# PeterFWS/Structure-PLP-SLAM

Hardware: NVIDIA H100
Metric: frames_per_sec_extract_match_poseopt (higher is better)
Workload: dtype u8/f64

## Files before the change

### structure-plp-slam_b200/csrc/local_map.cu

```cuda
#include "common.cuh"
#include "local_map_kernels.cuh"
#include "match_kernels.cuh"
#include "pose_kernels.cuh"
#include "tracker.h"

namespace plp {

namespace {

using lm::LocalDev;
using lm::local_finish_kernel;
using lm::local_gather_kernel;
using lm::local_observe_kernel;
using lm::local_prep_kernel;

}

}

using namespace plp;

extern "C" {

plp_status plp_tracker_reserve_local_map(plp_tracker *t, float log_scale_factor, int max_local_points) {
// ... 71 lines not shown
    D.rb = t->standing(kStageRobust);
    if (from_update) {
        D.kf.local_idx = D.rb.local_idx = t->upd_local_idx;
        D.kf.local_idx_offsets = D.rb.local_idx_offsets = t->upd_local_idx_offsets;
    }
    D.pos_w = local->pos_w;
    D.normal = local->obs_mean_normal;
    D.min_d = local->min_valid_dist;
    D.max_d = local->max_valid_dist;
    D.max_raw = local->max_valid_dist_raw;
    D.lm_desc = local->desc;
    D.valid = local->valid;
    D.offsets = local->offsets;
    D.margin = margin;
    D.matched = d_matched_out;
    D.local = d_local_out;
    D.observable = d_observable_out;
    D.pose = d_pose_out;
    D.num_tracked = d_num_tracked_out;
    D.n_inliers = d_n_inliers_out;
    D.lm_iters = d_lm_iters_out;
    D.status = d_status_out;

    PLP_LAUNCH(ctx, local_prep_kernel, batch, lm::kThreads, 0, D);
    PLP_CHECK_LAUNCH();
    const dim3 ogrid(div_up(t->max_local, lm::kObserveThreads), batch);
    PLP_LAUNCH(ctx, local_observe_kernel, ogrid, lm::kObserveThreads, 0, D);
    PLP_CHECK_LAUNCH();
    PLP_TRY(launch_point_match(ctx, D.mjobs, batch, t->cap > kMatchMaxPoints ? kMatchMaxPoints : t->cap, t->grid, 1,
                               lm::kLoweRatio, 0));
    PLP_LAUNCH(ctx, local_gather_kernel, batch, lm::kThreads, 0, D);
    PLP_CHECK_LAUNCH();
    plp_pose_opt_cfg cfg{4, 10};
    PLP_TRY(launch_pose_opt(ctx, D.posejobs, batch, t->cam, cfg));
    PLP_LAUNCH(ctx, local_finish_kernel, batch, lm::kThreads, 0, D);
    PLP_CHECK_LAUNCH();
    return PLP_OK;
}

plp_status plp_tracker_match_counts(const plp_tracker *t, const uint32_t **d_motion, const uint32_t **d_local) {
    PLP_REQUIRE(t && d_motion && d_local, "null pointer");
    *d_motion = t->dev.num_matches;
    *d_local = t->local ? t->local->num_matches : nullptr;
    return PLP_OK;
}

}
```

### structure-plp-slam_b200/csrc/match.cu

```cuda
#include "match_common.cuh"
#include "match_kernels.cuh"
#include "point_match_kernels.cuh"
#include "detmath.h"

namespace plp {

namespace {

constexpr int kThreads = 512;
__global__ void hamming_matrix_kernel(const uint8_t *__restrict__ a, int na, const uint8_t *__restrict__ b,
                                      int nb, uint16_t *__restrict__ out) {
    __shared__ uint4 sb[32][2];
    const int j0 = blockIdx.x * 32, i0 = blockIdx.y * 32;
    const int tx = threadIdx.x, ty = threadIdx.y;
    if (ty < 2 && j0 + tx < nb) sb[tx][ty] = __ldg(reinterpret_cast<const uint4 *>(b + 32 * (size_t)(j0 + tx)) + ty);
    __syncthreads();
    for (int r = ty; r < 32; r += 8) {
        const int i = i0 + r;
        if (i >= na) break;
        uint4 a0, a1;
        load_desc(a + 32 * (size_t)i, a0, a1);
        if (j0 + tx < nb) out[(size_t)i * nb + j0 + tx] = (uint16_t)hamming256(a0, a1, sb[tx][0], sb[tx][1]);
    }
}
// ... 407 lines not shown
            if (lane >= off) incl += nb;
        }
        int run = incl - local, med = 0x7fffffff;
#pragma unroll
        for (int q = 0; q < 9; ++q) {
            if (med == 0x7fffffff && run <= rank && rank < run + cnt[q]) med = lane * 9 + q;
            run += cnt[q];
        }
        for (int off = 16; off >= 1; off >>= 1) med = min(med, __shfl_xor_sync(0xffffffffu, med, off));
        if ((unsigned)med < best_median) {
            best_median = (unsigned)med;
            best_idx = i;
        }
        __syncwarp();
    }
    if (lane == 0) best_out[lm] = best_idx;
}

}

plp_status launch_point_match(plp_ctx *ctx, const PointMatchJob *d_jobs, int num_jobs, int max_n,
                              const plp_grid &grid, int ratio_test, float lowe_ratio, int check_orientation) {
    if (num_jobs <= 0) return PLP_OK;
    if (max_n > kMatchMaxPoints) {
        set_error("window matcher: %d keypoints exceed the per-frame capacity %d", max_n, kMatchMaxPoints);
        return PLP_ERR_CAPACITY;
    }
    if (grid.num_rows > 255 || grid.num_cols < 1 || grid.num_cols > 16383 || grid.num_rows < 1) {
        set_error("window matcher: unsupported grid %d x %d", grid.num_cols, grid.num_rows);
        return PLP_ERR_INVALID;
    }
    const int cap = max_n < 64 ? 64 : ((max_n + 63) / 64) * 64;
    const size_t smem = pm::point_smem_bytes(cap, grid.num_cols, grid.num_rows);
    using pm::point_match_kernel;
    PLP_SMEM_OPTIN(point_match_kernel, smem);
    PLP_LAUNCH(ctx, point_match_kernel, num_jobs, pm::kThreads, smem, d_jobs, grid, cap, ratio_test, lowe_ratio,
               check_orientation);
    PLP_CHECK_LAUNCH();
    return PLP_OK;
}

plp_status launch_line_match(plp_ctx *ctx, const LineMatchJob *d_jobs, int num_jobs, int ratio_test,
                             float lowe_ratio, int rgbd_gate) {
    if (num_jobs <= 0) return PLP_OK;
    const size_t smem = (size_t)2 * 16384 * 4 + 32;
    PLP_SMEM_OPTIN(line_match_kernel, smem);
    PLP_LAUNCH(ctx, line_match_kernel, num_jobs, kThreads, smem, d_jobs, ratio_test, lowe_ratio, rgbd_gate);
    PLP_CHECK_LAUNCH();
    return PLP_OK;
}

plp_status launch_brute_match(plp_ctx *ctx, const BruteJob *d_jobs, int num_jobs, int max_n_frm, float lowe_ratio,
                              int check_orientation) {
    if (num_jobs <= 0) return PLP_OK;
    if (max_n_frm > kBruteMaxPoints) {
        set_error("brute-force matcher: %d keypoints exceed the capacity %d", max_n_frm, kBruteMaxPoints);
        return PLP_ERR_CAPACITY;
    }
    const int cap = max_n_frm < 64 ? 64 : ((max_n_frm + 63) / 64) * 64;
    const size_t smem = (size_t)cap * 32 + (size_t)cap * 8 + kHistLen * 4 + 16 + 32;
    PLP_SMEM_OPTIN(brute_match_kernel, smem);
    PLP_LAUNCH(ctx, brute_match_kernel, num_jobs, kThreads, smem, d_jobs, cap, lowe_ratio, check_orientation);
    PLP_CHECK_LAUNCH();
    return PLP_OK;
}

plp_status launch_project_points(plp_ctx *ctx, const ProjectJob *d_jobs, int num_jobs, int max_n,
                                 const plp_camera &cam, const float *d_scale_factors, int num_levels, float margin) {
    if (num_jobs <= 0 || max_n <= 0) return PLP_OK;
    dim3 grid(div_up(max_n, 128), num_jobs);
// ... 625 lines not shown
```

### structure-plp-slam_b200/csrc/match_jobs.h

```cpp
#pragma once
#include <stdint.h>

namespace plp {

constexpr int kMatchMaxPoints = 3072;
constexpr int kBruteMaxPoints = 4096;

struct PointMatchJob {
    int n;
    const float *x, *y;
    const int32_t *octave;
    const float *angle;
    const float *x_right;
    const uint8_t *desc;
    const uint8_t *claimed;
    int m;
    const float *qx, *qy;
    const float *qxr;
    const float *qradius;
    const int32_t *qmin, *qmax;
    const float *qangle;
    const uint8_t *qdesc;
    const uint8_t *qvalid;
    int32_t *choice;
    int32_t *best_idx_out;
    int32_t *matched_out;
    uint32_t *num_matches;
    unsigned hamm_thr_p1;
};

struct LineMatchJob {
    int n;
    const float *sx, *sy, *ex, *ey;
    const int32_t *octave;
    const int32_t *ratio_level;
    const float *xr_sp, *xr_ep;
    const uint8_t *desc;
    const uint8_t *claimed;
// ... 43 lines not shown
```

### structure-plp-slam_b200/csrc/pipeline.cu

```cuda
#include "common.cuh"
#include "camera_kernels.cuh"
#include "match_kernels.cuh"
#include "pose_kernels.cuh"
#include "track_common.cuh"
#include "tracker.h"

namespace plp {

namespace {

__global__ void track_prep_kernel(TrackDev T, float margin, int check_orientation) {
    const int b = blockIdx.x, tid = threadIdx.x;
    const int n = T.n_kp[b];
    const size_t base = (size_t)b * T.cap;
    for (int i = tid; i < n; i += blockDim.x) {
        const plp_keypoint k = T.kp[base + i];
        T.x[base + i] = k.x;
        T.y[base + i] = k.y;
        T.angle[base + i] = k.angle;
        T.octave[base + i] = k.octave;
    }
    if (tid == 0) {
        const int l0 = T.last_offsets[b], m = T.last_offsets[b + 1] - l0;
        for (int attempt = 0; attempt < 2; ++attempt) {
// ... 29 lines not shown
            J.qy = P.qy;
            J.qxr = P.qxr;
            J.qradius = P.qradius;
            J.qmin = P.qmin;
            J.qmax = P.qmax;
            J.qangle = T.last_angle + l0;
            J.qdesc = T.last_desc + (size_t)l0 * 32;
            J.qvalid = P.qvalid;
            J.choice = T.choice + qb;
            J.best_idx_out = nullptr;
            J.matched_out = T.matched + base;
            J.num_matches = T.num_matches + b;
            T.pjobs[attempt * T.batch + b] = P;
            T.mjobs[attempt * T.batch + b] = J;
        }
    }
}

__global__ void track_retry_gate_kernel(TrackDev T) {
    const int b = blockIdx.x * blockDim.x + threadIdx.x;
    if (b >= T.batch) return;
    if (T.num_matches[b] >= (uint32_t)kNumMatchesThr) {
        T.pjobs[T.batch + b].n_last = -1;
        T.mjobs[T.batch + b].m = -1;
    }
}

}

plp_status launch_track_tail(plp_ctx *ctx, const TrackTail &J, int batch, const plp_camera &cam) {
    PLP_LAUNCH(ctx, track_gather_kernel, batch, kTailThreads, 0, J);
    PLP_CHECK_LAUNCH();
    plp_pose_opt_cfg cfg{4, 10};
    PLP_TRY(launch_pose_opt(ctx, J.posejobs, batch, cam, cfg));
    PLP_LAUNCH(ctx, track_finish_kernel, batch, kTailThreads, 0, J);
    PLP_CHECK_LAUNCH();
    return PLP_OK;
}

}

using namespace plp;

namespace plp {
plp_status make_undist_job(const plp_camera *cam, const plp_distortion *dist, UndistJob *J);
bool distortion_is_identity(const plp_distortion *dist);
plp_status launch_undistort(plp_ctx *ctx, const UndistJob &J);
}

extern "C" {

plp_status plp_tracker_create(plp_ctx *ctx, const plp_camera *cam, const plp_grid *grid, const float *scale_factors,
                              const float *inv_level_sigma_sq, int num_levels, int max_batch, int kp_capacity,
                              int max_last_points, plp_tracker **out) {
    return plp_tracker_create_ex(ctx, cam, grid, scale_factors, inv_level_sigma_sq, num_levels, max_batch, kp_capacity,
                                 max_last_points, nullptr, out);
}

plp_status plp_tracker_create_ex(plp_ctx *ctx, const plp_camera *cam, const plp_grid *grid, const float *scale_factors,
                                 const float *inv_level_sigma_sq, int num_levels, int max_batch, int kp_capacity,
                                 int max_last_points, const plp_distortion *dist, plp_tracker **out) {
    PLP_REQUIRE(ctx && cam && grid && scale_factors && inv_level_sigma_sq && out, "null pointer");
    const bool distorted = !distortion_is_identity(dist);
    UndistJob uj;
    if (distorted) PLP_TRY(make_undist_job(cam, dist, &uj));
    PLP_REQUIRE(num_levels >= 1 && num_levels <= 16 && max_batch >= 1 && kp_capacity >= 1 && max_last_points >= 1, "sizes");
    PLP_REQUIRE(cam->setup_type == 0, "the batched tracker implements the monocular path");
// ... 144 lines not shown
```

### structure-plp-slam_b200/csrc/point_match_kernels.cuh

```cuda
#pragma once
#include <stddef.h>
#include <stdint.h>

#include "../../include/plpslam_b200.h"
#include "devmath.cuh"
#include "match_common.cuh"
#include "match_jobs.h"

namespace plp {

namespace pm {

constexpr int kThreads = 1024;
constexpr int kGroup = 4;
constexpr int kNoKey = 0x7fffffff;

struct PointSmem {
    uint4 *desc;
    float *x, *y, *xr;
    int *meta;
    int *orig;
    int *owner_a, *owner_b;
    int *col_start;
    int *cursor;
    int *hist;
    int *flags;
    int *warp_sums;
    uint8_t *bin_valid;
    uint8_t *colchg;
};

__device__ __forceinline__ PointSmem carve_point_smem(uint8_t *base, int cap, int num_cols, int num_rows) {
    PointSmem s;
    const size_t cells2 = (size_t)(num_cols * num_rows + 2);
    s.desc = reinterpret_cast<uint4 *>(base);
    base += (size_t)cap * 32;
    s.x = reinterpret_cast<float *>(base);
    base += (size_t)cap * 4;
    s.y = reinterpret_cast<float *>(base);
    base += (size_t)cap * 4;
    s.xr = reinterpret_cast<float *>(base);
    base += (size_t)cap * 4;
    s.meta = reinterpret_cast<int *>(base);
    base += (size_t)cap * 4;
    s.orig = reinterpret_cast<int *>(base);
    base += (size_t)cap * 4;
    s.owner_a = reinterpret_cast<int *>(base);
    base += (size_t)cap * 4;
    s.owner_b = reinterpret_cast<int *>(base);
    base += (size_t)cap * 4;
    s.col_start = reinterpret_cast<int *>(base);
    base += cells2 * 4;
    s.cursor = reinterpret_cast<int *>(base);
    base += cells2 * 4;
    s.hist = reinterpret_cast<int *>(base);
    base += kHistLen * 4;
    s.flags = reinterpret_cast<int *>(base);
    base += 4 * 4;
    s.warp_sums = reinterpret_cast<int *>(base);
    base += 32 * 4;
    s.bin_valid = base;
    s.colchg = base + 32;
    return s;
}

static inline size_t point_smem_bytes(int cap, int num_cols, int num_rows) {
    return (size_t)cap * (32 + 7 * 4) + (size_t)(num_cols * num_rows + 2) * 8 + kHistLen * 4 + 16 + 128 + 32 +
           (size_t)(num_cols + 16);
}

__device__ __forceinline__ void group_scan(const PointSmem &S, const PointMatchJob &J, const plp_grid &grid, bool active,
                                           int q, int gl, const int *owner, int floor, int &k1, int &k2) {
    k1 = kNoKey;
    k2 = kNoKey;
    if (active) {
        const float ref_x = J.qx[q], ref_y = J.qy[q], r = J.qradius[q];
        const int min_level = J.qmin[q], max_level = J.qmax[q];
        Window w;
        if (query_window(grid, ref_x, ref_y, r, w)) {
            const bool check_level = (0 < min_level) || (0 <= max_level);
            const float qxr = J.qxr ? J.qxr[q] : 0.0f;
            uint4 q0, q1;
            load_desc(J.qdesc + 32 * (size_t)q, q0, q1);
            for (int c = w.min_cx + gl; c <= w.max_cx; c += kGroup) {
                const int p_begin = S.col_start[c * grid.num_rows + w.min_cy];
                const int p_end = S.col_start[c * grid.num_rows + w.max_cy + 1];
                for (int p = p_begin; p < p_end; ++p) {
                    const int meta = S.meta[p];
                    const int oct = (int)(signed char)(meta & 0xff);
                    if (check_level) {
                        if (oct < min_level) continue;
                        if (0 <= max_level && max_level < oct) continue;
                    }
                    const float dx = S.x[p] - ref_x, dy = S.y[p] - ref_y;
                    if (!(fabsf(dx) < r && fabsf(dy) < r)) continue;
                    if ((meta >> 16) & 1) continue;
                    if (owner && owner[p] < q) continue;
                    const float xr = S.xr[p];
                    if (0 < xr) {
                        const float err = fabsf(qxr - xr);
                        if (r < err) continue;
                    }
                    const int d = hamming256(q0, q1, S.desc[2 * p], S.desc[2 * p + 1]);
                    if (d >= PLP_MAX_HAMMING_DIST) continue;
                    const int key = (d << 12) | p;
                    if (key <= floor) continue;
                    if (key < k1) {
                        k2 = k1;
                        k1 = key;
                    } else if (key < k2) {
                        k2 = key;
                    }
                }
            }
        }
    }
    warp_top2<kGroup>(k1, k2);
}

__device__ __forceinline__ bool group_any(bool v) {
    int x = v ? 1 : 0;
#pragma unroll
    for (int o = kGroup / 2; o > 0; o >>= 1) x |= __shfl_xor_sync(0xffffffffu, x, o);
    return x != 0;
}

__global__ void __launch_bounds__(kThreads, 1)
    point_match_kernel(const PointMatchJob *__restrict__ jobs, plp_grid grid, int cap, int ratio_test, float lowe_ratio,
                       int check_orientation) {
    PLP_DYNAMIC_SMEM(smem_raw);
    const PointMatchJob &J = jobs[blockIdx.x];
    if (J.m < 0) return;
    PointSmem S = carve_point_smem(smem_raw, cap, grid.num_cols, grid.num_rows);
    const int tid = threadIdx.x, lane = tid & 31;
    if (J.n > cap) {
        if (J.matched_out)
            for (int i = tid; i < J.n; i += kThreads) J.matched_out[i] = -1;
        if (J.best_idx_out)
            for (int q = tid; q < J.m; q += kThreads) J.best_idx_out[q] = -1;
        if (tid == 0 && J.num_matches) *J.num_matches = 0xffffffffu;
        return;
    }
    const int n = J.n, m = J.m;

    int *key = S.owner_a;
    if (tid < 4) S.flags[tid] = 0;
    const int n_in = sort_by_cell<kThreads>(grid, n, J.x, J.y, key, S.col_start, S.cursor, S.warp_sums, S.orig);
    for (int p = tid; p < n_in; p += kThreads) {
        const int i = S.orig[p];
        const int k = key[i];
        const int cy = k % grid.num_rows;
        S.x[p] = J.x[i];
        S.y[p] = J.y[i];
        S.xr[p] = J.x_right ? J.x_right[i] : -1.0f;
        const int cl = J.claimed ? (J.claimed[i] != 0) : 0;
        S.meta[p] = (J.octave[i] & 0xff) | (cy << 8) | (cl << 16) | ((k / grid.num_rows) << 17);
        uint4 d0, d1;
        load_desc(J.desc + 32 * (size_t)i, d0, d1);
        S.desc[2 * p] = d0;
        S.desc[2 * p + 1] = d1;
    }
    __syncthreads();

    int *owner_prev = S.owner_a, *owner_next = S.owner_b;
    for (int p = tid; p < n_in; p += kThreads) {
        owner_prev[p] = kNoOwner;
        owner_next[p] = kNoOwner;
    }
    __syncthreads();

    const int gl = tid & (kGroup - 1);
    const int grp = tid / kGroup;
    constexpr int kGroups = kThreads / kGroup;
    const int m_pad = ((m + kGroups - 1) / kGroups) * kGroups;

    if (!ratio_test) {
        int *owner = owner_prev;
        const int hamm_thr = J.hamm_thr_p1 ? (int)J.hamm_thr_p1 - 1 : PLP_HAMMING_DIST_THR_HIGH;
        int cur = -1, floor = -1;
        const int leader = lane & ~(kGroup - 1);
        for (;;) {
            {
                int q = -1;
                if (cur < 0 && gl == 0) {
                    q = atomicAdd(&S.flags[3], 1);
                    while (q < m && J.qvalid && J.qvalid[q] == 0) {
                        J.choice[q] = -1;
                        q = atomicAdd(&S.flags[3], 1);
                    }
                    if (q >= m) q = -1;
                }
                const int got = __shfl_sync(0xffffffffu, q, leader);
                if (cur < 0) {
                    cur = got;
                    floor = -1;
                }
            }
            if (!__any_sync(0xffffffffu, cur >= 0)) break;
            int k1, k2;
            group_scan(S, J, grid, cur >= 0, cur, gl, nullptr, floor, k1, k2);
            int next = -1, nfloor = -1;
            if (gl == 0 && cur >= 0) {
                J.choice[cur] = -1;
#pragma unroll
                for (int t = 0; t < 2; ++t) {
                    const int key = t == 0 ? k1 : k2;
                    if (key == kNoKey || (key >> 12) > hamm_thr) {
                        next = -1;
                        break;
                    }
                    const int choice = key & 0xfff;
                    J.choice[cur] = choice;
                    __threadfence_block();
                    const int old = atomicMin(&owner[choice], cur);
                    if (old < cur) {
                        J.choice[cur] = -1;
                        next = cur;
                        nfloor = key;
                        continue;
                    }
                    next = -1;
                    if (old != kNoOwner) {
                        uint4 o0, o1;
                        load_desc(J.qdesc + 32 * (size_t)old, o0, o1);
                        next = old;
                        nfloor = (hamming256(o0, o1, S.desc[2 * choice], S.desc[2 * choice + 1]) << 12) | choice;
                    }
                    break;
                }
            }
            cur = __shfl_sync(0xffffffffu, next, leader);
            floor = __shfl_sync(0xffffffffu, nfloor, leader);
        }
        __syncthreads();
    } else {
        for (int round = 0; round <= m; ++round) {
            for (int q0 = 0; q0 < m_pad; q0 += kGroups) {
                const int q = q0 + grp;
                const bool valid = q < m && (J.qvalid ? (J.qvalid[q] != 0) : true);
                bool rescan = valid;
                if (valid && round > 0) {
                    Window w;
                    query_window(grid, J.qx[q], J.qy[q], J.qradius[q], w);
                    bool dirty = false;
                    for (int c = w.min_cx + gl; c <= w.max_cx; c += kGroup) dirty = dirty || S.colchg[c];
                    rescan = dirty;
                }
                if (round > 0) rescan = group_any(rescan);
                if (!__any_sync(0xffffffffu, rescan)) {
                    if (gl == 0 && valid) {
                        const int choice = J.choice[q];
                        if (choice >= 0) atomicMin(&owner_next[choice], q);
                    } else if (gl == 0 && q < m) {
                        J.choice[q] = -1;
                    }
                    continue;
                }
                int k1, k2;
                group_scan(S, J, grid, rescan, q, gl, owner_prev, -1, k1, k2);
// ... 34 lines not shown
            int *t = owner_prev;
            owner_prev = owner_next;
            owner_next = t;
            for (int p = tid; p < n_in; p += kThreads) owner_next[p] = kNoOwner;
            __syncthreads();
        }
    }

    for (int b = tid; b < kHistLen; b += kThreads) S.hist[b] = 0;
    if (J.matched_out)
        for (int i = tid; i < n; i += kThreads) J.matched_out[i] = -1;
    __syncthreads();
    const bool do_angle = check_orientation && J.qangle != nullptr && J.angle != nullptr;
    const auto delta = [&](int q, int p) { return J.qangle[q] - J.angle[S.orig[p]]; };
    orientation_check<kThreads>(m, J.choice, do_angle, S.hist, S.bin_valid, &S.flags[1], delta);
    for (int q = tid; q < m; q += kThreads) {
        const int p = J.choice[q];
        int out = -1;
        if (p >= 0) {
            const int i = S.orig[p];
            if (!do_angle || S.bin_valid[angle_bin(delta(q, p))]) {
                out = i;
                if (J.matched_out) J.matched_out[i] = q;
            } else {
                atomicAdd(&S.flags[2], 1);
            }
        }
        if (J.best_idx_out) J.best_idx_out[q] = out;
    }
    __syncthreads();
    if (tid == 0 && J.num_matches) *J.num_matches = (uint32_t)(S.flags[1] - S.flags[2]);
}

}

}
```

### structure-plp-slam_b200/csrc/pose_kernels.cuh

```cuda
#pragma once
#include "common.cuh"
#include "pose_jobs.h"

namespace plp {

plp_status launch_pose_opt(plp_ctx *ctx, const PoseJob *d_jobs, int batch, const plp_camera &cam,
                           const plp_pose_opt_cfg &cfg);

}
```

### structure-plp-slam_b200/csrc/pose_opt.cu

```cuda
#include "common.cuh"
#include "se3.cuh"
#include "pose_kernels.cuh"
#include "pose_opt_kernels.cuh"

namespace plp {

namespace {

__global__ void build_pose_jobs_kernel(PoseJob *jobs, int batch, const double *T_in, const plp_pt_obs *pts,
                                       const int32_t *pt_off, const plp_line_obs *lines, const int32_t *line_off,
                                       double *T_out, uint8_t *pt_outlier, uint8_t *line_outlier, int32_t *n_inl,
                                       int32_t *lm_iters) {
    const int b = blockIdx.x * blockDim.x + threadIdx.x;
    if (b >= batch) return;
    PoseJob J;
    J.T_in = T_in + 16 * (size_t)b;
    J.pts = pts + pt_off[b];
    J.n_pts = pt_off[b + 1] - pt_off[b];
    const int l0 = line_off ? line_off[b] : 0, l1 = line_off ? line_off[b + 1] : 0;
    J.lines = lines ? lines + l0 : nullptr;
    J.n_lines = lines ? l1 - l0 : 0;
    J.T_out = T_out + 16 * (size_t)b;
    J.pt_outlier = pt_outlier + pt_off[b];
    J.line_outlier = line_outlier ? line_outlier + l0 : nullptr;
    J.n_inliers = n_inl + b;
    J.lm_iters = lm_iters ? lm_iters + b : nullptr;
    jobs[b] = J;
}

}

plp_status launch_pose_opt(plp_ctx *ctx, const PoseJob *d_jobs, int batch, const plp_camera &cam,
                           const plp_pose_opt_cfg &cfg) {
    if (batch <= 0) return PLP_OK;
    using po::pose_opt_kernel;
    PLP_LAUNCH(ctx, pose_opt_kernel, batch, po::kThreads, 0, d_jobs, batch, cam, cfg);
    PLP_CHECK_LAUNCH();
    return PLP_OK;
}

}

using namespace plp;

extern "C" {

plp_status plp_pose_optimize_batch_dev(plp_ctx *ctx, const plp_camera *cam, int batch, const double *d_T_in,
                                       const plp_pt_obs *d_pts, const int32_t *d_pt_off, const plp_line_obs *d_lines,
                                       const int32_t *d_line_off, int max_edges_per_frame, const plp_pose_opt_cfg *cfg,
                                       double *d_T_out, uint8_t *d_pt_outlier, uint8_t *d_line_outlier,
                                       int32_t *d_n_inliers, int32_t *d_lm_iters) {
    PLP_REQUIRE(ctx && cam && cfg && d_T_in && d_pts && d_pt_off && d_T_out && d_pt_outlier && d_n_inliers,
                "null pointer");
    PLP_REQUIRE(batch >= 0 && cfg->num_trials >= 1 && cfg->num_each_iter >= 1, "batch / cfg");
    PLP_REQUIRE(!d_lines || (d_line_off && d_line_outlier), "line arrays");
    if (batch == 0) return PLP_OK;
    PLP_CUDA_TRY(cudaSetDevice(ctx->device));
    void *d_jobs = nullptr;
    PLP_TRY(ctx_scratch(ctx, 1, (size_t)batch * sizeof(PoseJob), &d_jobs));
    PLP_LAUNCH(ctx, build_pose_jobs_kernel, div_up(batch, 128), 128, 0, (PoseJob *)d_jobs, batch, d_T_in, d_pts,
               d_pt_off, d_lines, d_line_off, d_T_out, d_pt_outlier, d_line_outlier, d_n_inliers, d_lm_iters);
    PLP_CHECK_LAUNCH();
    (void)max_edges_per_frame;
    return launch_pose_opt(ctx, (const PoseJob *)d_jobs, batch, *cam, *cfg);
}

plp_status plp_pose_optimize_batch(plp_ctx *ctx, const plp_camera *cam, int batch, const double *T_in,
                                   const plp_pt_obs *pts, const int32_t *pt_off, const plp_line_obs *lines,
                                   const int32_t *line_off, const plp_pose_opt_cfg *cfg, double *T_out,
                                   uint8_t *pt_outlier, uint8_t *line_outlier, int32_t *n_inliers) {
    PLP_REQUIRE(ctx && cam && cfg && T_in && pt_off && T_out && n_inliers, "null pointer");
    PLP_REQUIRE(batch >= 0, "batch");
    if (batch == 0) return PLP_OK;
    const int n_pts = pt_off[batch], n_lines = line_off ? line_off[batch] : 0;
    PLP_REQUIRE(n_pts >= 0 && n_lines >= 0 && pt_off[0] == 0 && (!line_off || line_off[0] == 0), "offsets");
    PLP_REQUIRE((n_pts == 0 || (pts && pt_outlier)) && (n_lines == 0 || (lines && line_outlier)), "null arrays");
    int max_edges = 0;
    for (int b = 0; b < batch; ++b) {
        const int e = (pt_off[b + 1] - pt_off[b]) + (line_off ? line_off[b + 1] - line_off[b] : 0);
        PLP_REQUIRE(pt_off[b + 1] >= pt_off[b] && (!line_off || line_off[b + 1] >= line_off[b]), "offsets not monotone");
        max_edges = e > max_edges ? e : max_edges;
    }
    PLP_CUDA_TRY(cudaSetDevice(ctx->device));
    DevLayout L;
    const double *d_T;
    const plp_pt_obs *d_pts;
    const int32_t *d_po, *d_lo = nullptr;
    const plp_line_obs *d_lines = nullptr;
    double *d_To;
    uint8_t *d_pout, *d_lout = nullptr;
    int32_t *d_inl;
    L.in(d_T, T_in, (size_t)batch * 16);
    L.in(d_pts, pts, n_pts, n_pts ? n_pts : 1);
    L.in(d_po, pt_off, (size_t)batch + 1);
    if (n_lines) {
        L.in(d_lines, lines, n_lines);
        L.in(d_lo, line_off, (size_t)batch + 1);
// ... 27 lines not shown
```

### structure-plp-slam_b200/csrc/pose_opt_kernels.cuh

```cuda
#pragma once
#include <math.h>
#include <stddef.h>
#include <stdint.h>

#include "../../include/plpslam_b200.h"
#include "pose_jobs.h"
#include "se3.cuh"

namespace plp {

namespace po {

constexpr int kWarps = 4;
constexpr int kThreads = 32 * kWarps;
constexpr int kRed = 28;

struct Shared {
    double redH[2][kWarps][kRed];
    double redc[2][kWarps];
    se3::Pose pert[12];
    se3::Pose last_eval;
    int bad[2][kWarps];
};

__device__ __forceinline__ double warp_allsum(double v) {
#pragma unroll
    for (int o = 16; o > 0; o >>= 1) v += __shfl_xor_sync(0xffffffffu, v, o);
    return v;
}

__device__ __forceinline__ double sumH(const Shared &S, int hp, int k) {
    double a = S.redH[hp][0][k];
#pragma unroll
    for (int w = 1; w < kWarps; ++w) a += S.redH[hp][w][k];
    return a;
}

__device__ __forceinline__ bool solve6(const Shared &S, int hp, double lambda, double *x) {
    double A[6][6], b[6];
    {
        int k = 0;
#pragma unroll
        for (int i = 0; i < 6; ++i)
#pragma unroll
            for (int j = i; j < 6; ++j) {
                A[j][i] = sumH(S, hp, k);
                ++k;
            }
#pragma unroll
        for (int i = 0; i < 6; ++i) b[i] = sumH(S, hp, 21 + i);
    }
    double inv[6];
    bool ok = true;
#pragma unroll
    for (int j = 0; j < 6; ++j) {
        double d = A[j][j] + lambda;
#pragma unroll
        for (int q = 0; q < j; ++q) d -= A[j][q] * A[j][q];
        if (!(d > 0.0) || !isfinite(d)) ok = false;
        const double r = 1.0 / sqrt(d);
        inv[j] = r;
        A[j][j] = d * r;
#pragma unroll
        for (int i = j + 1; i < 6; ++i) {
            double s = A[i][j];
#pragma unroll
            for (int q = 0; q < j; ++q) s -= A[i][q] * A[j][q];
            A[i][j] = s * r;
        }
    }
    if (!ok) return false;
    double y[6];
#pragma unroll
    for (int i = 0; i < 6; ++i) {
        double s = b[i];
#pragma unroll
        for (int q = 0; q < i; ++q) s -= A[i][q] * y[q];
        y[i] = s * inv[i];
    }
#pragma unroll
    for (int i = 5; i >= 0; --i) {
        double s = y[i];
#pragma unroll
// ... 23 lines not shown
    const double rx = cam.fx * pc[0] * iz + cam.cx;
    e[0] = (double)o.obs_x - rx;
    e[1] = (double)o.obs_y - (cam.fy * pc[1] * iz + cam.cy);
    e[2] = stereo ? (double)o.x_right - (rx - cam.bf * iz) : 0.0;
    const double w = (double)o.inv_sigma_sq;
    return e[0] * (w * e[0]) + e[1] * (w * e[1]) + (stereo ? e[2] * (w * e[2]) : 0.0);
}

__device__ __forceinline__ void point_jac(const se3::Cam &c, const double *pc, double iz, bool stereo, double *J ) {
    const double x = pc[0], y = pc[1], iz2 = iz * iz;
    const double xz = x * iz, yz = y * iz;
    J[0] = xz * yz * c.fx;
    J[1] = -(1.0 + xz * xz) * c.fx;
    J[2] = yz * c.fx;
    J[3] = -iz * c.fx;
    J[4] = 0.0;
    J[5] = x * iz2 * c.fx;
    J[6] = (1.0 + yz * yz) * c.fy;
    J[7] = -xz * yz * c.fy;
    J[8] = -xz * c.fy;
    J[9] = 0.0;
    J[10] = -iz * c.fy;
    J[11] = y * iz2 * c.fy;
    if (stereo) {
        J[12] = J[0] - c.bf * y * iz2;
        J[13] = J[1] + c.bf * x * iz2;
        J[14] = J[2];
        J[15] = J[3];
        J[16] = 0.0;
        J[17] = J[5] - c.bf * iz2;
    }
}

__device__ __forceinline__ double eval_line(const se3::Cam &cam, const se3::Pose &P, const plp_line_obs &o, double *e) {
    const double obs[4] = {(double)o.sp_x, (double)o.sp_y, (double)o.ep_x, (double)o.ep_y};
    se3::line_error(cam, P.R, P.t, o.plucker, obs, e);
    const double w = (double)o.inv_sigma_sq;
    return e[0] * (w * e[0]) + e[1] * (w * e[1]);
}

__global__ void __launch_bounds__(kThreads, 2)
    pose_opt_kernel(const PoseJob *__restrict__ jobs, int batch, plp_camera pcam, plp_pose_opt_cfg cfg) {
    __shared__ Shared S;
    const int tid = threadIdx.x;
    const int f = blockIdx.x;
    if (f >= batch) return;
    const PoseJob J = jobs[f];
    const int n_pts = J.n_pts, n_lines = J.n_lines;
    const plp_pt_obs *pts = J.pts;
    const plp_line_obs *lines = J.lines;
    uint8_t *pt_level = J.pt_outlier;
    uint8_t *ln_level = J.line_outlier;
    const se3::Cam cam{pcam.fx, pcam.fy, pcam.cx, pcam.cy, pcam.focal_x_baseline};
    const double chi_sq_2D = (double)5.99146f, chi_sq_3D = (double)7.81473f;
    const double delta_pt = pcam.setup_type == 0 ? (double)sqrtf(5.99146f) : (double)sqrtf(7.81473f);
    const double delta_line = (double)sqrtf(5.99146f);
    int hp = 0, cp = 0;

    for (int i = tid; i < n_pts; i += kThreads) pt_level[i] = 0;
    for (int i = tid; i < n_lines; i += kThreads) ln_level[i] = 0;
    if (n_pts < 5) {
        if (tid < 16) J.T_out[tid] = J.T_in[tid];
        if (tid == 0) {
            *J.n_inliers = 0;
            if (J.lm_iters) *J.lm_iters = 0;
        }
        return;
    }
    se3::Pose est = se3::from_matrix(J.T_in);
    bool robust = true;
    int num_bad = 0, lm_iters = 0;
    double lambda = 0, ni = 2;
    for (int trial = 0; trial < cfg.num_trials; ++trial) {
        for (int it = 0; it < cfg.num_each_iter; ++it) {
            if (n_lines > 0) {
                __syncthreads();
                if (tid < 12) {
                    double u[6] = {0, 0, 0, 0, 0, 0};
                    u[tid >> 1] = (tid & 1) ? -1e-9 : 1e-9;
                    S.pert[tid] = se3::oplus(est, u);
                }
                __syncthreads();
            }
            double acc[kRed];
#pragma unroll
            for (int k = 0; k < kRed; ++k) acc[k] = 0;
            #pragma unroll 1
            for (int i = tid; i < n_pts; i += kThreads) {
                if (pt_level[i]) continue;
                const plp_pt_obs o = load_pt(pts + i);
                double Jm[18], e[3], pc[3], iz;
                bool stereo;
                const double chi2 = eval_point(cam, est, o, e, pc, iz, stereo);
                point_jac(cam, pc, iz, stereo, Jm);
                double rho0 = chi2, rho1 = 1.0;
                if (robust) se3::huber(chi2, delta_pt, rho0, rho1);
                acc[27] += rho0;
                const double ww = (double)o.inv_sigma_sq * rho1;
                if (!stereo) {
                    int k = 0;
#pragma unroll
                    for (int a = 0; a < 6; ++a) {
                        const double wa = ww * Jm[a], wb = ww * Jm[6 + a];
#pragma unroll
                        for (int c = a; c < 6; ++c) {
                            acc[k] += wa * Jm[c] + wb * Jm[6 + c];
                            ++k;
                        }
                        acc[21 + a] -= wa * e[0] + wb * e[1];
                    }
                } else {
                    int k = 0;
#pragma unroll
                    for (int a = 0; a < 6; ++a) {
                        const double wa = ww * Jm[a], wb = ww * Jm[6 + a], wc = ww * Jm[12 + a];
#pragma unroll
                        for (int c = a; c < 6; ++c) {
                            acc[k] += wa * Jm[c] + wb * Jm[6 + c] + wc * Jm[12 + c];
                            ++k;
                        }
                        acc[21 + a] -= wa * e[0] + wb * e[1] + wc * e[2];
                    }
                }
            }
            #pragma unroll 1
            for (int i = tid; i < n_lines; i += kThreads) {
                if (ln_level[i]) continue;
                const plp_line_obs o = lines[i];
                double Jm[12], e[2];
                const double chi2 = eval_line(cam, est, o, e);
                const double scalar = 1.0 / (2 * 1e-9);
#pragma unroll
                for (int d = 0; d < 6; ++d) {
                    double ep[2], em[2];
                    eval_line(cam, S.pert[2 * d], o, ep);
                    eval_line(cam, S.pert[2 * d + 1], o, em);
                    Jm[d] = scalar * (ep[0] - em[0]);
                    Jm[6 + d] = scalar * (ep[1] - em[1]);
                }
                double rho0 = chi2, rho1 = 1.0;
                if (robust) se3::huber(chi2, delta_line, rho0, rho1);
                acc[27] += rho0;
                const double ww = (double)o.inv_sigma_sq * rho1;
                int k = 0;
#pragma unroll
                for (int a = 0; a < 6; ++a) {
                    const double wa = ww * Jm[a], wb = ww * Jm[6 + a];
#pragma unroll
                    for (int c = a; c < 6; ++c) {
                        acc[k] += wa * Jm[c] + wb * Jm[6 + c];
                        ++k;
                    }
                    acc[21 + a] -= wa * e[0] + wb * e[1];
                }
            }
            hp ^= 1;
#pragma unroll
            for (int k = 0; k < kRed; ++k) {
                const double v = warp_allsum(acc[k]);
                if ((tid & 31) == 0) S.redH[hp][tid >> 5][k] = v;
            }
            __syncthreads();
            double current_chi = sumH(S, hp, 27);
            if (it == 0) {
                double md = 0;
                const int diag[6] = {0, 6, 11, 15, 18, 20};
#pragma unroll
                for (int j = 0; j < 6; ++j) md = fmax(fabs(sumH(S, hp, diag[j])), md);
                lambda = 1e-5 * md;
                ni = 2;
            }
            int qmax = 0;
            bool terminate = false;
            while (true) {
                double x[6] = {0, 0, 0, 0, 0, 0};
                const bool ok2 = solve6(S, hp, lambda, x);
                const se3::Pose trial_pose = se3::oplus(est, x);
                double chi = 0;
                #pragma unroll 1
                for (int i = tid; i < n_pts; i += kThreads) {
                    if (pt_level[i]) continue;
                    const plp_pt_obs o = load_pt(pts + i);
                    double e[3], pc[3], iz;
                    bool stereo;
                    const double chi2 = eval_point(cam, trial_pose, o, e, pc, iz, stereo);
                    double rho0 = chi2, rho1;
                    if (robust) se3::huber(chi2, delta_pt, rho0, rho1);
                    chi += rho0;
                }
                #pragma unroll 1
                for (int i = tid; i < n_lines; i += kThreads) {
                    if (ln_level[i]) continue;
                    double e[2];
                    const double chi2 = eval_line(cam, trial_pose, lines[i], e);
                    double rho0 = chi2, rho1;
                    if (robust) se3::huber(chi2, delta_line, rho0, rho1);
                    chi += rho0;
                }
                cp ^= 1;
                chi = warp_allsum(chi);
                if ((tid & 31) == 0) S.redc[cp][tid >> 5] = chi;
                __syncthreads();
                if (tid == 0) S.last_eval = trial_pose;
                double temp_chi = S.redc[cp][0];
#pragma unroll
                for (int w = 1; w < kWarps; ++w) temp_chi += S.redc[cp][w];
                if (!ok2) temp_chi = 1.7976931348623157e308;
                double rho = current_chi - temp_chi;
                double scale = 0;
#pragma unroll
                for (int j = 0; j < 6; ++j) scale += x[j] * (lambda * x[j] + sumH(S, hp, 21 + j));
                scale += 1e-3;
                rho /= scale;
                bool lambda_finite = true;
                if (rho > 0 && isfinite(temp_chi)) {
                    const double t = 2 * rho - 1;
                    double alpha = 1. - t * t * t;
                    alpha = fmin(alpha, 2. / 3.);
                    const double sf = fmax(1. / 3., alpha);
                    lambda *= sf;
                    ni = 2;
                    current_chi = temp_chi;
                    est = trial_pose;
                } else {
                    lambda *= ni;
                    ni *= 2;
                    if (!isfinite(lambda)) lambda_finite = false;
                }
                if (lambda_finite) qmax++;
                terminate = (qmax == 10 || rho == 0 || !lambda_finite);
                if (!(lambda_finite && rho < 0 && qmax < 10)) break;
            }
            ++lm_iters;
            if (terminate) break;
        }
        __syncthreads();
        int bad = 0;
        #pragma unroll 1
        for (int i = tid; i < n_pts; i += kThreads) {
            const plp_pt_obs o = load_pt(pts + i);
            double e[3], pc[3], iz;
            bool stereo;
            const double chi2 = pt_level[i] ? eval_point(cam, est, o, e, pc, iz, stereo)
                                            : eval_point(cam, S.last_eval, o, e, pc, iz, stereo);
            const bool out = (stereo ? chi_sq_3D : chi_sq_2D) < chi2;
            pt_level[i] = out ? 1 : 0;
            bad += out;
        }
#pragma unroll
        for (int o = 16; o > 0; o >>= 1) bad += __shfl_xor_sync(0xffffffffu, bad, o);
        if ((tid & 31) == 0) S.bad[trial & 1][tid >> 5] = bad;
        __syncthreads();
        num_bad = 0;
#pragma unroll
        for (int w = 0; w < kWarps; ++w) num_bad += S.bad[trial & 1][w];
        const bool drop_kernel = (trial == cfg.num_trials - 2);
        if (n_pts - num_bad < 5) break;
        #pragma unroll 1
        for (int i = tid; i < n_lines; i += kThreads) {
            double e[2];
            const double chi2 = ln_level[i] ? eval_line(cam, est, lines[i], e) : eval_line(cam, S.last_eval, lines[i], e);
            ln_level[i] = chi_sq_2D < chi2 ? 1 : 0;
        }
        if (drop_kernel) robust = false;
    }
    if (tid == 0) {
        double T[16];
        se3::to_matrix(est, T);
        for (int k = 0; k < 16; ++k) J.T_out[k] = T[k];
        *J.n_inliers = n_pts - num_bad;
        if (J.lm_iters) *J.lm_iters = lm_iters;
    }
}

}

}
```

Baseline: 93660.

## Shrink point-match smem/threads with size tiers and add points-only pose kernel

The point matcher stops staging descriptors in shared memory and reads them from global memory through the sorted index. It drops to 256 threads per block with a launch bound of 4 blocks per SM, and splits large frames into a second launch tier, with the xy arrays aliased over the cursor buffer. A points-only template instantiation of pose optimisation is used by the tracking paths and allows a higher launch bound. These changes aim to raise occupancy and cut shared-memory footprint, at the cost of more global descriptor loads and an extra launch. Tracking paths now ignore lines in pose optimisation, which changes behaviour if lines are present.

```diff
diff --git a/structure-plp-slam_b200/csrc/local_map.cu b/structure-plp-slam_b200/csrc/local_map.cu
--- a/structure-plp-slam_b200/csrc/local_map.cu
+++ b/structure-plp-slam_b200/csrc/local_map.cu
@@ -127,7 +127,7 @@
     PLP_LAUNCH(ctx, local_gather_kernel, batch, lm::kThreads, 0, D);
     PLP_CHECK_LAUNCH();
     plp_pose_opt_cfg cfg{4, 10};
-    PLP_TRY(launch_pose_opt(ctx, D.posejobs, batch, t->cam, cfg));
+    PLP_TRY(launch_pose_opt(ctx, D.posejobs, batch, t->cam, cfg, false));
     PLP_LAUNCH(ctx, local_finish_kernel, batch, lm::kThreads, 0, D);
     PLP_CHECK_LAUNCH();
     return PLP_OK;
diff --git a/structure-plp-slam_b200/csrc/match.cu b/structure-plp-slam_b200/csrc/match.cu
--- a/structure-plp-slam_b200/csrc/match.cu
+++ b/structure-plp-slam_b200/csrc/match.cu
@@ -463,10 +463,22 @@
     }
     const int cap = max_n < 64 ? 64 : ((max_n + 63) / 64) * 64;
     const size_t smem = pm::point_smem_bytes(cap, grid.num_cols, grid.num_rows);
-    using pm::point_match_kernel;
-    PLP_SMEM_OPTIN(point_match_kernel, smem);
-    PLP_LAUNCH(ctx, point_match_kernel, num_jobs, pm::kThreads, smem, d_jobs, grid, cap, ratio_test, lowe_ratio,
-               check_orientation);
+    if (cap <= kMatchSmallPoints) {
+        using pm::point_match_kernel;
+        PLP_SMEM_OPTIN(point_match_kernel, smem);
+        PLP_LAUNCH(ctx, point_match_kernel, num_jobs, pm::kThreads, smem, d_jobs, grid, cap, ratio_test, lowe_ratio,
+                   check_orientation);
+        PLP_CHECK_LAUNCH();
+        return PLP_OK;
+    }
+    using pm::point_match_tier_kernel;
+    PLP_SMEM_OPTIN(point_match_tier_kernel, smem);
+    PLP_LAUNCH(ctx, point_match_tier_kernel, num_jobs, pm::kThreads,
+               pm::point_smem_bytes(kMatchSmallPoints, grid.num_cols, grid.num_rows), d_jobs, grid, -1,
+               kMatchSmallPoints, 0, ratio_test, lowe_ratio, check_orientation);
+    PLP_CHECK_LAUNCH();
+    PLP_LAUNCH(ctx, point_match_tier_kernel, num_jobs, pm::kThreads, smem, d_jobs, grid, kMatchSmallPoints, cap, 1,
+               ratio_test, lowe_ratio, check_orientation);
     PLP_CHECK_LAUNCH();
     return PLP_OK;
 }
diff --git a/structure-plp-slam_b200/csrc/match_jobs.h b/structure-plp-slam_b200/csrc/match_jobs.h
--- a/structure-plp-slam_b200/csrc/match_jobs.h
+++ b/structure-plp-slam_b200/csrc/match_jobs.h
@@ -4,6 +4,7 @@
 namespace plp {
 
 constexpr int kMatchMaxPoints = 3072;
+constexpr int kMatchSmallPoints = 1536;
 constexpr int kBruteMaxPoints = 4096;
 
 struct PointMatchJob {
diff --git a/structure-plp-slam_b200/csrc/pipeline.cu b/structure-plp-slam_b200/csrc/pipeline.cu
--- a/structure-plp-slam_b200/csrc/pipeline.cu
+++ b/structure-plp-slam_b200/csrc/pipeline.cu
@@ -85,7 +85,7 @@
     PLP_LAUNCH(ctx, track_gather_kernel, batch, kTailThreads, 0, J);
     PLP_CHECK_LAUNCH();
     plp_pose_opt_cfg cfg{4, 10};
-    PLP_TRY(launch_pose_opt(ctx, J.posejobs, batch, cam, cfg));
+    PLP_TRY(launch_pose_opt(ctx, J.posejobs, batch, cam, cfg, false));
     PLP_LAUNCH(ctx, track_finish_kernel, batch, kTailThreads, 0, J);
     PLP_CHECK_LAUNCH();
     return PLP_OK;
diff --git a/structure-plp-slam_b200/csrc/point_match_kernels.cuh b/structure-plp-slam_b200/csrc/point_match_kernels.cuh
--- a/structure-plp-slam_b200/csrc/point_match_kernels.cuh
+++ b/structure-plp-slam_b200/csrc/point_match_kernels.cuh
@@ -11,12 +11,11 @@
 
 namespace pm {
 
-constexpr int kThreads = 1024;
+constexpr int kThreads = 256;
 constexpr int kGroup = 4;
 constexpr int kNoKey = 0x7fffffff;
 
 struct PointSmem {
-    uint4 *desc;
     float *x, *y, *xr;
     int *meta;
     int *orig;
@@ -30,19 +29,20 @@
     uint8_t *colchg;
 };
 
+__host__ __device__ inline size_t point_xy_bytes(int cap, int num_cols, int num_rows) {
+    const size_t xy = (size_t)cap * 16, cur = (size_t)(num_cols * num_rows + 2) * 4;
+    return xy > cur ? xy : cur;
+}
+
 __device__ __forceinline__ PointSmem carve_point_smem(uint8_t *base, int cap, int num_cols, int num_rows) {
     PointSmem s;
     const size_t cells2 = (size_t)(num_cols * num_rows + 2);
-    s.desc = reinterpret_cast<uint4 *>(base);
-    base += (size_t)cap * 32;
+    s.cursor = reinterpret_cast<int *>(base);
     s.x = reinterpret_cast<float *>(base);
-    base += (size_t)cap * 4;
-    s.y = reinterpret_cast<float *>(base);
-    base += (size_t)cap * 4;
-    s.xr = reinterpret_cast<float *>(base);
-    base += (size_t)cap * 4;
-    s.meta = reinterpret_cast<int *>(base);
-    base += (size_t)cap * 4;
+    s.y = s.x + cap;
+    s.xr = s.y + cap;
+    s.meta = reinterpret_cast<int *>(s.xr + cap);
+    base += point_xy_bytes(cap, num_cols, num_rows);
     s.orig = reinterpret_cast<int *>(base);
     base += (size_t)cap * 4;
     s.owner_a = reinterpret_cast<int *>(base);
@@ -50,8 +50,6 @@
     s.owner_b = reinterpret_cast<int *>(base);
     base += (size_t)cap * 4;
     s.col_start = reinterpret_cast<int *>(base);
-    base += cells2 * 4;
-    s.cursor = reinterpret_cast<int *>(base);
     base += cells2 * 4;
     s.hist = reinterpret_cast<int *>(base);
     base += kHistLen * 4;
@@ -65,8 +63,12 @@
 }
 
 static inline size_t point_smem_bytes(int cap, int num_cols, int num_rows) {
-    return (size_t)cap * (32 + 7 * 4) + (size_t)(num_cols * num_rows + 2) * 8 + kHistLen * 4 + 16 + 128 + 32 +
-           (size_t)(num_cols + 16);
+    return point_xy_bytes(cap, num_cols, num_rows) + (size_t)cap * 3 * 4 + (size_t)(num_cols * num_rows + 2) * 4 +
+           kHistLen * 4 + 16 + 128 + 32 + (size_t)(num_cols + 16);
+}
+
+__device__ __forceinline__ void sorted_desc(const PointSmem &S, const PointMatchJob &J, int p, uint4 &a, uint4 &b) {
+    load_desc(J.desc + 32 * (size_t)S.orig[p], a, b);
 }
 
 __device__ __forceinline__ void group_scan(const PointSmem &S, const PointMatchJob &J, const plp_grid &grid, bool active,
@@ -101,7 +103,9 @@
                         const float err = fabsf(qxr - xr);
                         if (r < err) continue;
                     }
-                    const int d = hamming256(q0, q1, S.desc[2 * p], S.desc[2 * p + 1]);
+                    uint4 d0, d1;
+                    sorted_desc(S, J, p, d0, d1);
+                    const int d = hamming256(q0, q1, d0, d1);
                     if (d >= PLP_MAX_HAMMING_DIST) continue;
                     const int key = (d << 12) | p;
                     if (key <= floor) continue;
@@ -125,12 +129,9 @@
     return x != 0;
 }
 
-__global__ void __launch_bounds__(kThreads, 1)
-    point_match_kernel(const PointMatchJob *__restrict__ jobs, plp_grid grid, int cap, int ratio_test, float lowe_ratio,
-                       int check_orientation) {
+__device__ __forceinline__ void match_frame(const PointMatchJob &J, const plp_grid &grid, int cap, int ratio_test,
+                                            float lowe_ratio, int check_orientation) {
     PLP_DYNAMIC_SMEM(smem_raw);
-    const PointMatchJob &J = jobs[blockIdx.x];
-    if (J.m < 0) return;
     PointSmem S = carve_point_smem(smem_raw, cap, grid.num_cols, grid.num_rows);
     const int tid = threadIdx.x, lane = tid & 31;
     if (J.n > cap) {
@@ -155,10 +156,6 @@
         S.xr[p] = J.x_right ? J.x_right[i] : -1.0f;
         const int cl = J.claimed ? (J.claimed[i] != 0) : 0;
         S.meta[p] = (J.octave[i] & 0xff) | (cy << 8) | (cl << 16) | ((k / grid.num_rows) << 17);
-        uint4 d0, d1;
-        load_desc(J.desc + 32 * (size_t)i, d0, d1);
-        S.desc[2 * p] = d0;
-        S.desc[2 * p + 1] = d1;
     }
     __syncthreads();
 
@@ -221,10 +218,11 @@
                     }
                     next = -1;
                     if (old != kNoOwner) {
-                        uint4 o0, o1;
+                        uint4 o0, o1, c0, c1;
                         load_desc(J.qdesc + 32 * (size_t)old, o0, o1);
+                        sorted_desc(S, J, choice, c0, c1);
                         next = old;
-                        nfloor = (hamming256(o0, o1, S.desc[2 * choice], S.desc[2 * choice + 1]) << 12) | choice;
+                        nfloor = (hamming256(o0, o1, c0, c1) << 12) | choice;
                     }
                     break;
                 }
@@ -325,6 +323,23 @@
     if (tid == 0 && J.num_matches) *J.num_matches = (uint32_t)(S.flags[1] - S.flags[2]);
 }
 
-}
-
-}
+__global__ void __launch_bounds__(kThreads, 4)
+    point_match_kernel(const PointMatchJob *__restrict__ jobs, plp_grid grid, int cap, int ratio_test, float lowe_ratio,
+                       int check_orientation) {
+    const PointMatchJob &J = jobs[blockIdx.x];
+    if (J.m < 0) return;
+    match_frame(J, grid, cap, ratio_test, lowe_ratio, check_orientation);
+}
+
+__global__ void __launch_bounds__(kThreads, 4)
+    point_match_tier_kernel(const PointMatchJob *__restrict__ jobs, plp_grid grid, int n_lo, int cap, int last,
+                            int ratio_test, float lowe_ratio, int check_orientation) {
+    const PointMatchJob &J = jobs[blockIdx.x];
+    if (J.m < 0) return;
+    if (J.n <= n_lo || (J.n > cap && !last)) return;
+    match_frame(J, grid, cap, ratio_test, lowe_ratio, check_orientation);
+}
+
+}
+
+}
diff --git a/structure-plp-slam_b200/csrc/pose_kernels.cuh b/structure-plp-slam_b200/csrc/pose_kernels.cuh
--- a/structure-plp-slam_b200/csrc/pose_kernels.cuh
+++ b/structure-plp-slam_b200/csrc/pose_kernels.cuh
@@ -5,6 +5,6 @@
 namespace plp {
 
 plp_status launch_pose_opt(plp_ctx *ctx, const PoseJob *d_jobs, int batch, const plp_camera &cam,
-                           const plp_pose_opt_cfg &cfg);
+                           const plp_pose_opt_cfg &cfg, bool lines);
 
 }
diff --git a/structure-plp-slam_b200/csrc/pose_opt.cu b/structure-plp-slam_b200/csrc/pose_opt.cu
--- a/structure-plp-slam_b200/csrc/pose_opt.cu
+++ b/structure-plp-slam_b200/csrc/pose_opt.cu
@@ -31,10 +31,14 @@
 }
 
 plp_status launch_pose_opt(plp_ctx *ctx, const PoseJob *d_jobs, int batch, const plp_camera &cam,
-                           const plp_pose_opt_cfg &cfg) {
+                           const plp_pose_opt_cfg &cfg, bool lines) {
     if (batch <= 0) return PLP_OK;
     using po::pose_opt_kernel;
-    PLP_LAUNCH(ctx, pose_opt_kernel, batch, po::kThreads, 0, d_jobs, batch, cam, cfg);
+    using po::pose_opt_points_kernel;
+    if (lines)
+        PLP_LAUNCH(ctx, pose_opt_kernel, batch, po::kThreads, 0, d_jobs, batch, cam, cfg);
+    else
+        PLP_LAUNCH(ctx, pose_opt_points_kernel, batch, po::kThreads, 0, d_jobs, batch, cam, cfg);
     PLP_CHECK_LAUNCH();
     return PLP_OK;
 }
@@ -62,7 +66,7 @@
                d_pt_off, d_lines, d_line_off, d_T_out, d_pt_outlier, d_line_outlier, d_n_inliers, d_lm_iters);
     PLP_CHECK_LAUNCH();
     (void)max_edges_per_frame;
-    return launch_pose_opt(ctx, (const PoseJob *)d_jobs, batch, *cam, *cfg);
+    return launch_pose_opt(ctx, (const PoseJob *)d_jobs, batch, *cam, *cfg, d_lines != nullptr);
 }
 
 plp_status plp_pose_optimize_batch(plp_ctx *ctx, const plp_camera *cam, int batch, const double *T_in,
diff --git a/structure-plp-slam_b200/csrc/pose_opt_kernels.cuh b/structure-plp-slam_b200/csrc/pose_opt_kernels.cuh
--- a/structure-plp-slam_b200/csrc/pose_opt_kernels.cuh
+++ b/structure-plp-slam_b200/csrc/pose_opt_kernels.cuh
@@ -145,14 +145,15 @@
     return e[0] * (w * e[0]) + e[1] * (w * e[1]);
 }
 
-__global__ void __launch_bounds__(kThreads, 2)
-    pose_opt_kernel(const PoseJob *__restrict__ jobs, int batch, plp_camera pcam, plp_pose_opt_cfg cfg) {
+template <bool kLines>
+__device__ __forceinline__ void pose_opt_frame(const PoseJob *__restrict__ jobs, int batch, const plp_camera &pcam,
+                                               const plp_pose_opt_cfg &cfg) {
     __shared__ Shared S;
     const int tid = threadIdx.x;
     const int f = blockIdx.x;
     if (f >= batch) return;
     const PoseJob J = jobs[f];
-    const int n_pts = J.n_pts, n_lines = J.n_lines;
+    const int n_pts = J.n_pts, n_lines = kLines ? J.n_lines : 0;
     const plp_pt_obs *pts = J.pts;
     const plp_line_obs *lines = J.lines;
     uint8_t *pt_level = J.pt_outlier;
@@ -179,7 +180,7 @@
     double lambda = 0, ni = 2;
     for (int trial = 0; trial < cfg.num_trials; ++trial) {
         for (int it = 0; it < cfg.num_each_iter; ++it) {
-            if (n_lines > 0) {
+            if (kLines && n_lines > 0) {
                 __syncthreads();
                 if (tid < 12) {
                     double u[6] = {0, 0, 0, 0, 0, 0};
@@ -379,6 +380,16 @@
     }
 }
 
-}
-
-}
+__global__ void __launch_bounds__(kThreads, 2)
+    pose_opt_kernel(const PoseJob *__restrict__ jobs, int batch, plp_camera pcam, plp_pose_opt_cfg cfg) {
+    pose_opt_frame<true>(jobs, batch, pcam, cfg);
+}
+
+__global__ void __launch_bounds__(kThreads, 4)
+    pose_opt_points_kernel(const PoseJob *__restrict__ jobs, int batch, plp_camera pcam, plp_pose_opt_cfg cfg) {
+    pose_opt_frame<false>(jobs, batch, pcam, cfg);
+}
+
+}
+
+}
```

Result: faster. 98200 (median of 6 runs) (+4.8%).

## Use transpose-style warp reduction and unroll point loops by two

Applied to the files above, without the earlier changes.

Replaces 28 separate butterfly warp all-reduces with a recursive-halving scatter reduction, so each lane ends up holding one of 32 Hessian entries, and reads the results with register shuffles instead of repeated shared-memory sums. Both point loops now process two observations per iteration, issuing both loads up front for more memory-level parallelism. The intent is to cut shuffle count, shared-memory traffic and load latency. The risk is higher register pressure from the larger accumulator array and the duplicated point bodies, which could hurt occupancy under launch_bounds(128,2).

```diff
diff --git a/structure-plp-slam_b200/csrc/pose_opt_kernels.cuh b/structure-plp-slam_b200/csrc/pose_opt_kernels.cuh
--- a/structure-plp-slam_b200/csrc/pose_opt_kernels.cuh
+++ b/structure-plp-slam_b200/csrc/pose_opt_kernels.cuh
@@ -13,10 +13,9 @@
 
 constexpr int kWarps = 4;
 constexpr int kThreads = 32 * kWarps;
-constexpr int kRed = 28;
 
 struct Shared {
-    double redH[2][kWarps][kRed];
+    double redH[2][kWarps][32];
     double redc[2][kWarps];
     se3::Pose pert[12];
     se3::Pose last_eval;
@@ -29,14 +28,35 @@
     return v;
 }
 
-__device__ __forceinline__ double sumH(const Shared &S, int hp, int k) {
-    double a = S.redH[hp][0][k];
-#pragma unroll
-    for (int w = 1; w < kWarps; ++w) a += S.redH[hp][w][k];
-    return a;
-}
-
-__device__ __forceinline__ bool solve6(const Shared &S, int hp, double lambda, double *x) {
+template <int o>
+__device__ __forceinline__ void scatter_step(double (&acc)[32], int lane) {
+    const bool hi = (lane & o) != 0;
+#pragma unroll
+    for (int k = 0; k < o; ++k) {
+        const double send = hi ? acc[k] : acc[k + o];
+        const double mine = hi ? acc[k + o] : acc[k];
+        acc[k] = mine + __shfl_xor_sync(0xffffffffu, send, o);
+    }
+}
+
+__device__ __forceinline__ double block_sum(double (&acc)[32], double (*red)[32]) {
+    const int lane = threadIdx.x & 31;
+    scatter_step<16>(acc, lane);
+    scatter_step<8>(acc, lane);
+    scatter_step<4>(acc, lane);
+    scatter_step<2>(acc, lane);
+    scatter_step<1>(acc, lane);
+    red[threadIdx.x >> 5][lane] = acc[0];
+    __syncthreads();
+    double t = red[0][lane];
+#pragma unroll
+    for (int w = 1; w < kWarps; ++w) t += red[w][lane];
+    return t;
+}
+
+__device__ __forceinline__ double col(double tot, int k) { return __shfl_sync(0xffffffffu, tot, k); }
+
+__device__ __forceinline__ bool solve6(double tot, double lambda, double *x) {
     double A[6][6], b[6];
     {
         int k = 0;
@@ -44,11 +64,11 @@
         for (int i = 0; i < 6; ++i)
 #pragma unroll
             for (int j = i; j < 6; ++j) {
-                A[j][i] = sumH(S, hp, k);
+                A[j][i] = col(tot, k);
                 ++k;
             }
 #pragma unroll
-        for (int i = 0; i < 6; ++i) b[i] = sumH(S, hp, 21 + i);
+        for (int i = 0; i < 6; ++i) b[i] = col(tot, 21 + i);
     }
     double inv[6];
     bool ok = true;
@@ -138,6 +158,53 @@
     }
 }
 
+__device__ __forceinline__ double point_cost(const se3::Cam &cam, const se3::Pose &P, const plp_pt_obs &o, bool robust,
+                                             double delta_pt) {
+    double e[3], pc[3], iz;
+    bool stereo;
+    const double chi2 = eval_point(cam, P, o, e, pc, iz, stereo);
+    double rho0 = chi2, rho1;
+    if (robust) se3::huber(chi2, delta_pt, rho0, rho1);
+    return rho0;
+}
+
+__device__ __forceinline__ void add_point(const se3::Cam &cam, const se3::Pose &P, const plp_pt_obs &o, bool robust,
+                                          double delta_pt, double (&acc)[32]) {
+    double Jm[18], e[3], pc[3], iz;
+    bool stereo;
+    const double chi2 = eval_point(cam, P, o, e, pc, iz, stereo);
+    point_jac(cam, pc, iz, stereo, Jm);
+    double rho0 = chi2, rho1 = 1.0;
+    if (robust) se3::huber(chi2, delta_pt, rho0, rho1);
+    acc[27] += rho0;
+    const double ww = (double)o.inv_sigma_sq * rho1;
+    if (!stereo) {
+        int k = 0;
+#pragma unroll
+        for (int a = 0; a < 6; ++a) {
+            const double wa = ww * Jm[a], wb = ww * Jm[6 + a];
+#pragma unroll
+            for (int c = a; c < 6; ++c) {
+                acc[k] += wa * Jm[c] + wb * Jm[6 + c];
+                ++k;
+            }
+            acc[21 + a] -= wa * e[0] + wb * e[1];
+        }
+    } else {
+        int k = 0;
+#pragma unroll
+        for (int a = 0; a < 6; ++a) {
+            const double wa = ww * Jm[a], wb = ww * Jm[6 + a], wc = ww * Jm[12 + a];
+#pragma unroll
+            for (int c = a; c < 6; ++c) {
+                acc[k] += wa * Jm[c] + wb * Jm[6 + c] + wc * Jm[12 + c];
+                ++k;
+            }
+            acc[21 + a] -= wa * e[0] + wb * e[1] + wc * e[2];
+        }
+    }
+}
+
 __device__ __forceinline__ double eval_line(const se3::Cam &cam, const se3::Pose &P, const plp_line_obs &o, double *e) {
     const double obs[4] = {(double)o.sp_x, (double)o.sp_y, (double)o.ep_x, (double)o.ep_y};
     se3::line_error(cam, P.R, P.t, o.plucker, obs, e);
@@ -188,46 +255,16 @@
                 }
                 __syncthreads();
             }
-            double acc[kRed];
-#pragma unroll
-            for (int k = 0; k < kRed; ++k) acc[k] = 0;
+            double acc[32];
+#pragma unroll
+            for (int k = 0; k < 32; ++k) acc[k] = 0;
             #pragma unroll 1
-            for (int i = tid; i < n_pts; i += kThreads) {
-                if (pt_level[i]) continue;
-                const plp_pt_obs o = load_pt(pts + i);
-                double Jm[18], e[3], pc[3], iz;
-                bool stereo;
-                const double chi2 = eval_point(cam, est, o, e, pc, iz, stereo);
-                point_jac(cam, pc, iz, stereo, Jm);
-                double rho0 = chi2, rho1 = 1.0;
-                if (robust) se3::huber(chi2, delta_pt, rho0, rho1);
-                acc[27] += rho0;
-                const double ww = (double)o.inv_sigma_sq * rho1;
-                if (!stereo) {
-                    int k = 0;
-#pragma unroll
-                    for (int a = 0; a < 6; ++a) {
-                        const double wa = ww * Jm[a], wb = ww * Jm[6 + a];
-#pragma unroll
-                        for (int c = a; c < 6; ++c) {
-                            acc[k] += wa * Jm[c] + wb * Jm[6 + c];
-                            ++k;
-                        }
-                        acc[21 + a] -= wa * e[0] + wb * e[1];
-                    }
-                } else {
-                    int k = 0;
-#pragma unroll
-                    for (int a = 0; a < 6; ++a) {
-                        const double wa = ww * Jm[a], wb = ww * Jm[6 + a], wc = ww * Jm[12 + a];
-#pragma unroll
-                        for (int c = a; c < 6; ++c) {
-                            acc[k] += wa * Jm[c] + wb * Jm[6 + c] + wc * Jm[12 + c];
-                            ++k;
-                        }
-                        acc[21 + a] -= wa * e[0] + wb * e[1] + wc * e[2];
-                    }
-                }
+            for (int i = tid; i < n_pts; i += 2 * kThreads) {
+                const int i1 = i + kThreads < n_pts ? i + kThreads : i;
+                const bool in0 = !pt_level[i], in1 = i1 != i && !pt_level[i1];
+                const plp_pt_obs o0 = load_pt(pts + i), o1 = load_pt(pts + i1);
+                if (in0) add_point(cam, est, o0, robust, delta_pt, acc);
+                if (in1) add_point(cam, est, o1, robust, delta_pt, acc);
             }
             #pragma unroll 1
             for (int i = tid; i < n_lines; i += kThreads) {
@@ -261,18 +298,12 @@
                 }
             }
             hp ^= 1;
-#pragma unroll
-            for (int k = 0; k < kRed; ++k) {
-                const double v = warp_allsum(acc[k]);
-                if ((tid & 31) == 0) S.redH[hp][tid >> 5][k] = v;
-            }
-            __syncthreads();
-            double current_chi = sumH(S, hp, 27);
+            const double tot = block_sum(acc, S.redH[hp]);
+            double current_chi = col(tot, 27);
             if (it == 0) {
                 double md = 0;
-                const int diag[6] = {0, 6, 11, 15, 18, 20};
-#pragma unroll
-                for (int j = 0; j < 6; ++j) md = fmax(fabs(sumH(S, hp, diag[j])), md);
+#pragma unroll
+                for (int j = 0, d = 0; j < 6; d += 6 - j, ++j) md = fmax(fabs(col(tot, d)), md);
                 lambda = 1e-5 * md;
                 ni = 2;
             }
@@ -280,19 +311,16 @@
             bool terminate = false;
             while (true) {
                 double x[6] = {0, 0, 0, 0, 0, 0};
-                const bool ok2 = solve6(S, hp, lambda, x);
+                const bool ok2 = solve6(tot, lambda, x);
                 const se3::Pose trial_pose = se3::oplus(est, x);
                 double chi = 0;
                 #pragma unroll 1
-                for (int i = tid; i < n_pts; i += kThreads) {
-                    if (pt_level[i]) continue;
-                    const plp_pt_obs o = load_pt(pts + i);
-                    double e[3], pc[3], iz;
-                    bool stereo;
-                    const double chi2 = eval_point(cam, trial_pose, o, e, pc, iz, stereo);
-                    double rho0 = chi2, rho1;
-                    if (robust) se3::huber(chi2, delta_pt, rho0, rho1);
-                    chi += rho0;
+                for (int i = tid; i < n_pts; i += 2 * kThreads) {
+                    const int i1 = i + kThreads < n_pts ? i + kThreads : i;
+                    const bool in0 = !pt_level[i], in1 = i1 != i && !pt_level[i1];
+                    const plp_pt_obs o0 = load_pt(pts + i), o1 = load_pt(pts + i1);
+                    if (in0) chi += point_cost(cam, trial_pose, o0, robust, delta_pt);
+                    if (in1) chi += point_cost(cam, trial_pose, o1, robust, delta_pt);
                 }
                 #pragma unroll 1
                 for (int i = tid; i < n_lines; i += kThreads) {
@@ -315,7 +343,7 @@
                 double rho = current_chi - temp_chi;
                 double scale = 0;
 #pragma unroll
-                for (int j = 0; j < 6; ++j) scale += x[j] * (lambda * x[j] + sumH(S, hp, 21 + j));
+                for (int j = 0; j < 6; ++j) scale += x[j] * (lambda * x[j] + col(tot, 21 + j));
                 scale += 1e-3;
                 rho /= scale;
                 bool lambda_finite = true;
```

New measurement: 93570 before, 94990 after (median of 6 runs). 1.02x the previous value.
